# Manta-Network/Plonk-Prototype

Hardware: NVIDIA B200
Metric: PLONK prove time (BLS12-381 / KZG10, synthetic arithmetic circuit, 2^20 gates) (lower is better)
Workload: dtype u32 limbs (Fr 8x32, Fp 12x32)

## Files before the change

include/pb200.h:

```cpp
#ifndef PB200_H
#define PB200_H
#include <stddef.h>
#include <stdint.h>

#if defined(__GNUC__)
#define PB200_API __attribute__((visibility("default")))
#else
#define PB200_API
#endif

#ifdef __cplusplus
extern "C" {
#endif

typedef struct pb200_ctx pb200_ctx;
typedef struct pb200_srs pb200_srs;

enum {
    PB200_OK = 0,
    PB200_ERR_ARG = 1,
    PB200_ERR_CUDA = 2,
    PB200_ERR_NO_DEVICE = 3
};

PB200_API int pb200_init(pb200_ctx **out, int device_id);
PB200_API void pb200_destroy(pb200_ctx *ctx);
PB200_API const char *pb200_last_error(const pb200_ctx *ctx);
PB200_API void *pb200_stream(pb200_ctx *ctx);
PB200_API int pb200_sync(pb200_ctx *ctx);

PB200_API int pb200_malloc(pb200_ctx *ctx, void **dev_ptr, size_t bytes);
PB200_API int pb200_free(pb200_ctx *ctx, void *dev_ptr);
PB200_API int pb200_h2d(pb200_ctx *ctx, void *dev_dst, const void *host_src, size_t bytes);
PB200_API int pb200_d2h(pb200_ctx *ctx, void *host_dst, const void *dev_src, size_t bytes);

PB200_API int pb200_domain_log_size(size_t num_coeffs, uint32_t *log_n);
PB200_API int pb200_ntt(pb200_ctx *ctx, uint64_t *data_host, uint32_t log_n, int inverse, int coset);
PB200_API int pb200_ntt_dev(pb200_ctx *ctx, uint64_t *data_dev, uint32_t log_n, int inverse, int coset);

PB200_API int pb200_ntt_batch_dev(pb200_ctx *ctx, uint64_t *data_dev, uint32_t log_n, uint32_t batch, int inverse, int coset);
PB200_API int pb200_ntt_columns_dev(pb200_ctx *ctx, uint64_t *data_dev, uint32_t log_n, uint32_t log_n1, uint32_t log_cols,
                                    uint32_t col_offset, int inverse);
PB200_API int pb200_ntt_columns_scatter_dev(pb200_ctx *ctx, uint64_t *data_dev, uint32_t log_n, uint32_t log_n1, uint32_t log_cols,
                                            uint32_t col_offset, uint32_t world, void *const *peer_row_bufs);
PB200_API int pb200_ipc_export(pb200_ctx *ctx, void *dev_ptr, unsigned char handle_out[64]);
PB200_API int pb200_ipc_open(pb200_ctx *ctx, const unsigned char handle[64], void **dev_ptr_out);
PB200_API int pb200_ipc_close(pb200_ctx *ctx, void *dev_ptr);
PB200_API int pb200_block_transpose_dev(pb200_ctx *ctx, uint64_t *dst_dev, const uint64_t *src_dev, uint32_t blocks,
                                        uint32_t rows, uint32_t cols);

PB200_API int pb200_srs_upload(pb200_ctx *ctx, const uint64_t *xy_mont_host, size_t n_points, pb200_srs **out);
PB200_API int pb200_srs_wrap_dev(pb200_ctx *ctx, const uint64_t *xy_mont_dev, size_t n_points, pb200_srs **out);
PB200_API int pb200_srs_precompute(pb200_ctx *ctx, pb200_srs *srs);
PB200_API void pb200_srs_free(pb200_ctx *ctx, pb200_srs *srs);
PB200_API size_t pb200_srs_len(const pb200_srs *srs);
PB200_API int pb200_msm_g1(pb200_ctx *ctx, const pb200_srs *srs, size_t offset, const uint64_t *scalars_mont_host, size_t n,
                 uint64_t out_xyz_mont[18]);
PB200_API int pb200_msm_g1_dev(pb200_ctx *ctx, const pb200_srs *srs, size_t offset, const uint64_t *scalars_mont_dev, size_t n,
                     uint64_t out_xyz_mont[18]);
PB200_API int pb200_msm_g1_batch_dev(pb200_ctx *ctx, const pb200_srs *srs, size_t offset, const uint64_t *scalars_mont_dev, size_t n,
                                     uint32_t batch, size_t scalar_stride, uint64_t *out_xyz_mont);
PB200_API int pb200_pippenger_g1(pb200_ctx *ctx, const uint64_t *points_xyz_mont_host, const uint64_t *scalars_mont_host, size_t n,
                                 uint64_t out_xyz_mont[18]);
PB200_API int pb200_g1_sum(pb200_ctx *ctx, const uint64_t *points_xyz_mont_host, size_t count, uint64_t out_xyz_mont[18]);
PB200_API uint32_t pb200_msm_window_bits(size_t n);

PB200_API int pb200_srs_generate(pb200_ctx *ctx, const uint64_t tau_mont[4], size_t n_points, pb200_srs **out);
PB200_API int pb200_srs_generate_range(pb200_ctx *ctx, const uint64_t tau_mont[4], size_t first, size_t n_points, pb200_srs **out);
PB200_API const uint64_t *pb200_srs_dev_ptr(const pb200_srs *srs);
enum {
    PB200_G1_OK = 0,
    PB200_G1_BAD_FLAGS = 1,
    PB200_G1_X_RANGE = 2,
    PB200_G1_NOT_ON_CURVE = 3,
    PB200_G1_NOT_IN_SUBGROUP = 4,
    PB200_G1_IDENTITY = 5
};
PB200_API int pb200_srs_from_compressed(pb200_ctx *ctx, const uint8_t *bytes_host, size_t n_points, uint8_t *status_host,
                                        pb200_srs **out);
PB200_API int pb200_srs_to_compressed(pb200_ctx *ctx, const pb200_srs *srs, size_t offset, size_t n, uint8_t *bytes_host);
PB200_API int pb200_kzg_witness_dev(pb200_ctx *ctx, const uint64_t *poly_dev, size_t n, const uint64_t z_mont[4],
                                    uint64_t *quotient_dev, uint64_t eval_mont_out[4]);
PB200_API int pb200_fr_horner_step_dev(pb200_ctx *ctx, uint64_t *acc_dev, size_t n_acc, const uint64_t *poly_dev, size_t n_poly,
                                       const uint64_t c_mont[4]);

typedef struct pb200_prover_key pb200_prover_key;
// ... 69 lines not shown
```

plonk-prototype_b200/_native.py:

```python
import ctypes
import os

import numpy as np

_HERE = os.path.dirname(os.path.abspath(__file__))
LIB_PATH = os.path.join(_HERE, "libpb200.so")
_lib = None

EXPORTS = [
    "pb200_init", "pb200_destroy", "pb200_last_error", "pb200_stream", "pb200_sync",
    "pb200_malloc", "pb200_free", "pb200_h2d", "pb200_d2h",
    "pb200_domain_log_size", "pb200_ntt", "pb200_ntt_dev", "pb200_ntt_batch_dev", "pb200_ntt_columns_dev", "pb200_ntt_columns_scatter_dev",
    "pb200_ipc_export", "pb200_ipc_open", "pb200_ipc_close", "pb200_block_transpose_dev",
    "pb200_srs_upload", "pb200_srs_wrap_dev", "pb200_srs_precompute", "pb200_srs_free", "pb200_srs_len",
    "pb200_msm_g1", "pb200_msm_g1_dev", "pb200_msm_g1_batch_dev", "pb200_pippenger_g1", "pb200_g1_sum", "pb200_msm_window_bits",
    "pb200_srs_generate", "pb200_srs_generate_range", "pb200_srs_dev_ptr", "pb200_kzg_witness_dev", "pb200_fr_horner_step_dev",
    "pb200_srs_from_compressed", "pb200_srs_to_compressed",
    "pb200_preprocess", "pb200_preprocess_sharded", "pb200_prover_key_free", "pb200_prover_key_size", "pb200_prover_key_bytes", "pb200_prove", "pb200_prove_dev",
    "pb200_transcript_selftest", "pb200_synthetic_circuit", "pb200_verify", "pb200_verify_batch", "pb200_opening_key_from_tau",
    "pb200_pairing_selftest",
    "pb200_synthetic_bases_dev", "pb200_profile_enable", "pb200_profile_ms", "pb200_profile_reset", "pb200_profile_sum_ms",
    "pb200_launch_count",
    "pb200_imad_peak",
    "pb200_comm_unique_id", "pb200_comm_init", "pb200_comm_destroy", "pb200_comm_info", "pb200_allgather_dev", "pb200_alltoall_dev",
    "pb200_msm_g1_sharded_dev", "pb200_ntt_sharded_dev", "pb200_preprocess_comm",
]


class Pb200Error(RuntimeError):
    pass


G1_OK, G1_BAD_FLAGS, G1_X_RANGE, G1_NOT_ON_CURVE, G1_NOT_IN_SUBGROUP, G1_IDENTITY = range(6)


ALLGATHER_FN = ctypes.CFUNCTYPE(ctypes.c_int, ctypes.c_void_p, ctypes.c_void_p, ctypes.c_void_p, ctypes.c_size_t)
DEV_COLLECTIVE_FN = ctypes.CFUNCTYPE(ctypes.c_int, ctypes.c_void_p, ctypes.c_void_p, ctypes.c_void_p, ctypes.c_size_t)


class Shard(ctypes.Structure):
    _fields_ = [("rank", ctypes.c_uint32), ("world", ctypes.c_uint32), ("allgather", ALLGATHER_FN), ("user", ctypes.c_void_p),
                ("alltoall_dev", DEV_COLLECTIVE_FN), ("allgather_dev", DEV_COLLECTIVE_FN), ("flags", ctypes.c_uint32)]


class Circuit(ctypes.Structure):
    _fields_ = [("n_gates", ctypes.c_size_t), ("n_vars", ctypes.c_size_t), ("selectors", ctypes.c_void_p * 11),
                ("wires", ctypes.c_void_p * 4)]
# ... 3 lines not shown
    global _lib
    if _lib is None:
        if not os.path.exists(LIB_PATH):
            raise Pb200Error("libpb200.so is not built (run `python -c 'import __graft_entry__ as g; g.build()'`); "
                             "there is no CPU fallback")
        L = ctypes.CDLL(LIB_PATH)
        vp, u64p = ctypes.c_void_p, ctypes.c_void_p
        L.pb200_init.argtypes = [ctypes.POINTER(vp), ctypes.c_int]
        L.pb200_destroy.argtypes = [vp]
        L.pb200_destroy.restype = None
        L.pb200_last_error.argtypes = [vp]
        L.pb200_last_error.restype = ctypes.c_char_p
        L.pb200_stream.argtypes = [vp]
        L.pb200_stream.restype = vp
        L.pb200_sync.argtypes = [vp]
        L.pb200_malloc.argtypes = [vp, ctypes.POINTER(vp), ctypes.c_size_t]
        L.pb200_free.argtypes = [vp, vp]
        L.pb200_h2d.argtypes = [vp, vp, vp, ctypes.c_size_t]
        L.pb200_d2h.argtypes = [vp, vp, vp, ctypes.c_size_t]
        L.pb200_domain_log_size.argtypes = [ctypes.c_size_t, ctypes.POINTER(ctypes.c_uint32)]
        L.pb200_ntt.argtypes = [vp, u64p, ctypes.c_uint32, ctypes.c_int, ctypes.c_int]
        L.pb200_ntt_dev.argtypes = [vp, u64p, ctypes.c_uint32, ctypes.c_int, ctypes.c_int]
        L.pb200_ntt_batch_dev.argtypes = [vp, u64p, ctypes.c_uint32, ctypes.c_uint32, ctypes.c_int, ctypes.c_int]
        L.pb200_ntt_columns_dev.argtypes = [vp, u64p, ctypes.c_uint32, ctypes.c_uint32, ctypes.c_uint32, ctypes.c_uint32, ctypes.c_int]
        L.pb200_ntt_columns_scatter_dev.argtypes = [vp, u64p, ctypes.c_uint32, ctypes.c_uint32, ctypes.c_uint32, ctypes.c_uint32,
                                                    ctypes.c_uint32, ctypes.POINTER(vp)]
        L.pb200_ipc_export.argtypes = [vp, vp, ctypes.c_char_p]
        L.pb200_ipc_open.argtypes = [vp, ctypes.c_char_p, ctypes.POINTER(vp)]
        L.pb200_ipc_close.argtypes = [vp, vp]
        L.pb200_block_transpose_dev.argtypes = [vp, u64p, u64p, ctypes.c_uint32, ctypes.c_uint32, ctypes.c_uint32]
        L.pb200_srs_upload.argtypes = [vp, u64p, ctypes.c_size_t, ctypes.POINTER(vp)]
        L.pb200_srs_wrap_dev.argtypes = [vp, u64p, ctypes.c_size_t, ctypes.POINTER(vp)]
        L.pb200_srs_precompute.argtypes = [vp, vp]
        L.pb200_srs_free.argtypes = [vp, vp]
        L.pb200_srs_free.restype = None
        L.pb200_srs_len.argtypes = [vp]
        L.pb200_srs_len.restype = ctypes.c_size_t
        L.pb200_msm_g1.argtypes = [vp, vp, ctypes.c_size_t, u64p, ctypes.c_size_t, u64p]
        L.pb200_msm_g1_dev.argtypes = [vp, vp, ctypes.c_size_t, u64p, ctypes.c_size_t, u64p]
        L.pb200_msm_g1_batch_dev.argtypes = [vp, vp, ctypes.c_size_t, u64p, ctypes.c_size_t, ctypes.c_uint32, ctypes.c_size_t, u64p]
        L.pb200_g1_sum.argtypes = [vp, u64p, ctypes.c_size_t, u64p]
        L.pb200_pippenger_g1.argtypes = [vp, u64p, u64p, ctypes.c_size_t, u64p]
        L.pb200_msm_window_bits.argtypes = [ctypes.c_size_t]
        L.pb200_msm_window_bits.restype = ctypes.c_uint32
        L.pb200_srs_generate.argtypes = [vp, u64p, ctypes.c_size_t, ctypes.POINTER(vp)]
        L.pb200_srs_dev_ptr.argtypes = [vp]
        L.pb200_srs_dev_ptr.restype = vp
        L.pb200_kzg_witness_dev.argtypes = [vp, u64p, ctypes.c_size_t, u64p, u64p, u64p]
        L.pb200_fr_horner_step_dev.argtypes = [vp, u64p, ctypes.c_size_t, u64p, ctypes.c_size_t, u64p]
        L.pb200_preprocess.argtypes = [vp, vp, ctypes.POINTER(Circuit), ctypes.c_char_p, ctypes.c_size_t, ctypes.POINTER(vp), vp]
        L.pb200_preprocess_sharded.argtypes = [vp, vp, ctypes.POINTER(Circuit), ctypes.c_char_p, ctypes.c_size_t, ctypes.POINTER(Shard),
                                               ctypes.POINTER(vp), vp]
        L.pb200_srs_generate_range.argtypes = [vp, u64p, ctypes.c_size_t, ctypes.c_size_t, ctypes.POINTER(vp)]
        L.pb200_srs_from_compressed.argtypes = [vp, vp, ctypes.c_size_t, vp, ctypes.POINTER(vp)]
        L.pb200_srs_to_compressed.argtypes = [vp, vp, ctypes.c_size_t, ctypes.c_size_t, vp]
        L.pb200_prover_key_free.argtypes = [vp, vp]
        L.pb200_prover_key_free.restype = None
        L.pb200_prover_key_size.argtypes = [vp]
        L.pb200_prover_key_size.restype = ctypes.c_size_t
        L.pb200_prover_key_bytes.argtypes = [vp]
        L.pb200_prover_key_bytes.restype = ctypes.c_size_t
        L.pb200_prove.argtypes = [vp, vp, vp, u64p, vp, u64p, ctypes.c_size_t, vp]
        L.pb200_prove_dev.argtypes = [vp, vp, vp, u64p, vp, u64p, ctypes.c_size_t, vp]
        L.pb200_transcript_selftest.argtypes = [ctypes.c_char_p, ctypes.c_char_p, ctypes.c_char_p, ctypes.c_size_t, ctypes.c_char_p,
                                                ctypes.c_char_p, ctypes.c_size_t]
        L.pb200_verify.argtypes = [vp, ctypes.c_size_t, ctypes.c_char_p, ctypes.c_size_t, vp, vp, u64p, ctypes.c_size_t, u64p,
# ... 143 lines not shown
        self._check(lib().pb200_ntt_columns_scatter_dev(self._h, ctypes.c_void_p(dev), log_n, log_n1, log_cols, col_offset,
                                                        len(peer_row_bufs), arr))

    def ipc_export(self, dev):
        buf = ctypes.create_string_buffer(64)
        self._check(lib().pb200_ipc_export(self._h, ctypes.c_void_p(dev), buf))
        return buf.raw

    def ipc_open(self, handle):
        p = ctypes.c_void_p()
        self._check(lib().pb200_ipc_open(self._h, handle, ctypes.byref(p)))
        return p.value

    def ipc_close(self, dev):
        self._check(lib().pb200_ipc_close(self._h, ctypes.c_void_p(dev)))

    def block_transpose_dev(self, dst, src, blocks, rows, cols):
        self._check(lib().pb200_block_transpose_dev(self._h, ctypes.c_void_p(dst), ctypes.c_void_p(src), blocks, rows, cols))

    def srs_upload(self, xy_host):
        assert xy_host.dtype == np.uint64 and xy_host.size % 12 == 0
        h = ctypes.c_void_p()
        self._check(lib().pb200_srs_upload(self._h, _ptr(xy_host), xy_host.size // 12, ctypes.byref(h)))
        return h

    def srs_wrap_dev(self, dev, n):
        h = ctypes.c_void_p()
        self._check(lib().pb200_srs_wrap_dev(self._h, ctypes.c_void_p(dev), n, ctypes.byref(h)))
        return h

    def srs_precompute(self, srs):
        self._check(lib().pb200_srs_precompute(self._h, srs))

    def srs_free(self, srs):
        lib().pb200_srs_free(self._h, srs)

    def msm(self, srs, scalars_host, offset=0):
        n = scalars_host.size // 4
        out = np.zeros(18, np.uint64)
        self._check(lib().pb200_msm_g1(self._h, srs, offset, _ptr(scalars_host), n, _ptr(out)))
        return out

    def msm_dev(self, srs, scalars_dev, n, offset=0):
        out = np.zeros(18, np.uint64)
        self._check(lib().pb200_msm_g1_dev(self._h, srs, offset, ctypes.c_void_p(scalars_dev), n, _ptr(out)))
        return out

    def msm_batch_dev(self, srs, scalars_dev, n, batch, stride, offset=0):
        out = np.zeros((batch, 18), np.uint64)
        self._check(lib().pb200_msm_g1_batch_dev(self._h, srs, offset, ctypes.c_void_p(scalars_dev), n, batch, stride, _ptr(out)))
        return out

    def pippenger(self, points_xyz_host, scalars_host):
        pts = np.ascontiguousarray(points_xyz_host, dtype=np.uint64).reshape(-1, 18)
        sc = np.ascontiguousarray(scalars_host, dtype=np.uint64).reshape(-1, 4)
        assert pts.shape[0] == sc.shape[0]
        out = np.zeros(18, np.uint64)
        self._check(lib().pb200_pippenger_g1(self._h, _ptr(pts) if pts.size else None, _ptr(sc) if sc.size else None, pts.shape[0], _ptr(out)))
        return out

    def g1_sum(self, points_xyz_host):
        pts = np.ascontiguousarray(points_xyz_host, dtype=np.uint64).reshape(-1, 18)
        out = np.zeros(18, np.uint64)
        self._check(lib().pb200_g1_sum(self._h, _ptr(pts), pts.shape[0], _ptr(out)))
        return out

# ... 220 lines not shown
```

plonk-prototype_b200/csrc/common.cuh:

```cuda
#pragma once
#include <cuda_runtime.h>
#include <stdint.h>
#include <stdio.h>

#include <map>
#include <string>
#include <vector>

#include "../../include/pb200.h"

struct NttPlan;
struct pb200_comm;

struct pb200_ctx {
    int device = 0;
    int sm_count = 0;
    cudaStream_t stream = nullptr;
    std::string err;
    uint64_t launches = 0;
    bool profile = false;
    std::map<std::string, float> prof_ms;
    std::map<std::string, float> prof_sum;
    std::map<std::string, uint32_t> prof_cnt;
    std::map<uint32_t, NttPlan *> ntt_plans;
// ... 62 lines not shown
    void collect() {
        if (a && b) {
            float ms = 0;
            if (cudaEventElapsedTime(&ms, a, b) == cudaSuccess) {
                ctx->prof_ms[name] = ms;
                ctx->prof_sum[name] += ms;
                ctx->prof_cnt[name]++;
            }
            cudaEventDestroy(a);
            cudaEventDestroy(b);
            a = b = nullptr;
        }
    }
    ~PbTimer() {
        if (a) cudaEventDestroy(a);
        if (b) cudaEventDestroy(b);
    }
};

int pb_ensure(pb200_ctx *ctx, void **buf, size_t *have, size_t need);
int comm_allgather_host(pb200_ctx *ctx, const void *send, void *recv, size_t bytes);
int comm_stream_barrier(pb200_ctx *ctx);
uint32_t *comm_partials_buffer(pb200_ctx *ctx);
int comm_sum_partials(pb200_ctx *ctx, uint32_t batch, uint64_t *out_xyz_host);
struct pb200_srs;
int msm_batch_to_dev(pb200_ctx *ctx, const pb200_srs *srs, size_t offset, const uint64_t *scalars_dev, size_t n, uint32_t batch,
                     size_t scalar_stride, uint32_t *result_dev, bool *handled);
int tail_g1_sum_batch(pb200_ctx *ctx, const uint32_t *pts, uint32_t count, uint32_t batch, uint32_t *results);
int kzg_witness_slice_phase1(pb200_ctx *ctx, const uint64_t *poly_slice_dev, uint32_t lo, uint32_t cnt, const uint64_t z_mont[4],
                             uint64_t *q_slice_dev, uint64_t *work_dev, uint64_t slice_total_out[4]);
int kzg_witness_slice_phase2(pb200_ctx *ctx, uint32_t lo, uint32_t cnt, uint64_t *q_slice_dev, uint64_t *work_dev,
                             const uint64_t later_slices_total[4]);
size_t kzg_witness_slice_work_scalars(uint32_t cnt);
```

plonk-prototype_b200/csrc/host_field.h:

```cpp
#pragma once
#include <stdint.h>
#include <string.h>

namespace hostf {

typedef unsigned __int128 u128;

template <int N>
struct Params;

template <>
struct Params<4> {
    static constexpr uint64_t MOD[4] = {0xffffffff00000001ull, 0x53bda402fffe5bfeull, 0x3339d80809a1d805ull, 0x73eda753299d7d48ull};
    static constexpr uint64_t INV = 0xfffffffeffffffffull;
    static constexpr uint64_t R2[4] = {0xc999e990f3f29c6dull, 0x2b6cedcb87925c23ull, 0x05d314967254398full, 0x0748d9d99f59ff11ull};
};
template <>
struct Params<6> {
    static constexpr uint64_t MOD[6] = {0xb9feffffffffaaabull, 0x1eabfffeb153ffffull, 0x6730d2a0f6b0f624ull,
                                        0x64774b84f38512bfull, 0x4b1ba7b6434bacd7ull, 0x1a0111ea397fe69aull};
    static constexpr uint64_t INV = 0x89f3fffcfffcfffdull;
    static constexpr uint64_t R2[6] = {0xf4df1f341c341746ull, 0x0a76e6a609d104f1ull, 0x8de5476c4c95b6d5ull,
                                       0x67eb88a9939d83c0ull, 0x9a793e85b519952dull, 0x11988fe592cae3aaull};
};
// ... 98 lines not shown
                t[j - 1] = (uint64_t)c;
                c >>= 64;
            }
            c += t[N];
            t[N - 1] = (uint64_t)c;
            t[N] = t[N + 1] + (uint64_t)(c >> 64);
        }
        El r;
        memcpy(r.l, t, sizeof(r.l));
        if (t[N] || geq_mod(r.l)) sub_mod(r.l);
        return r;
    }
    El sqr() const { return *this * *this; }
    El from_mont() const { return *this * raw_u64(1); }
    El pow(const uint64_t *e, int words) const {
        El r = one();
        for (int i = words * 64 - 1; i >= 0; i--) {
            r = r.sqr();
            if ((e[i >> 6] >> (i & 63)) & 1) r = r * *this;
        }
        return r;
    }
    El pow_u64(uint64_t e) const { return pow(&e, 1); }
    El inv() const {
        uint64_t e[N];
        for (int i = 0; i < N; i++) e[i] = P::MOD[i];
        e[0] -= 2;
        return pow(e, N);
    }
};
typedef El<4> HFr;
typedef El<6> HFp;

inline void fr_to_bytes(const HFr &a, uint8_t out[32]) {
    HFr c = a.from_mont();
    for (int i = 0; i < 4; i++)
        for (int k = 0; k < 8; k++) out[8 * i + k] = (uint8_t)(c.l[i] >> (8 * k));
}
inline HFr fr_from_bytes_wide(const uint8_t in[64]) {
    HFr lo, hi;
    for (int i = 0; i < 4; i++) {
        lo.l[i] = hi.l[i] = 0;
        for (int k = 7; k >= 0; k--) {
            lo.l[i] = (lo.l[i] << 8) | in[8 * i + k];
            hi.l[i] = (hi.l[i] << 8) | in[32 + 8 * i + k];
        }
    }
    const HFr r2 = HFr::r2(), r3 = r2 * r2;
    return lo * r2 + hi * r3;
}
inline void g1_projective_to_bytes(const uint64_t xyz[18], uint8_t out[48]) {
    HFp X = HFp::load(xyz), Y = HFp::load(xyz + 6), Z = HFp::load(xyz + 12);
    memset(out, 0, 48);
    if (Z.is_zero()) {
        out[0] = 0xc0;
        return;
    }
    HFp zi = Z.inv();
    HFp x = (X * zi).from_mont(), y = (Y * zi).from_mont();
    for (int i = 0; i < 6; i++)
        for (int k = 0; k < 8; k++) out[47 - (8 * i + k)] = (uint8_t)(x.l[i] >> (8 * k));
    uint64_t d[7];
    uint64_t c = 0;
    for (int i = 0; i < 6; i++) {
        d[i] = (y.l[i] << 1) | c;
        c = y.l[i] >> 63;
// ... 7 lines not shown
```

plonk-prototype_b200/csrc/plonk.cu:

```cuda
#include <algorithm>
#include <chrono>
#include <cstdlib>
#include <cstring>
#include <vector>

#include "common.cuh"
#include "fr_vec.cuh"
#include "host_field.h"
#include "merlin.h"
#include "widgets.h"

using hostf::HFr;

namespace {

constexpr int kSel = 11;
enum { Q_M, Q_L, Q_R, Q_O, Q_C, Q_4, Q_ARITH, Q_RANGE, Q_LOGIC, Q_FIXED, Q_VAR };
const char *const kSelLabel[kSel] = {"q_m", "q_l", "q_r", "q_o", "q_c", "q_4", "q_arith", "q_range", "q_logic",
                                     "q_fixed_group_add", "q_variable_group_add"};
const int kSeedOrder[kSel] = {Q_M, Q_L, Q_R, Q_O, Q_C, Q_4, Q_ARITH, Q_RANGE, Q_LOGIC, Q_VAR, Q_FIXED};

inline Fr to_dev(const HFr &h) {
    Fr r;
    memcpy(r.l, h.l, 32);
// ... 301 lines not shown
    if (first < len) {
        const uint32_t last = min(first + kEvalPerThread, len);
        acc = ld_fr(p + last - 1);
        for (uint32_t j = last - 1; j-- > first;) acc = acc * x + ld_fr(p + j);
        acc = acc * x.pow_u32(A.off[job] + first);
    }
    acc = block_sum(acc, sm);
    if (threadIdx.x == 0) st_fr(A.partial + (size_t)job * A.tiles + blockIdx.x, acc);
}
__global__ void __launch_bounds__(256) poly_eval_final_kernel(const Fr *partial, uint32_t tiles, Fr *out) {
    __shared__ uint4 smraw[512];
    Fr *sm = reinterpret_cast<Fr *>(smraw);
    const uint32_t job = blockIdx.x;
    Fr acc = Fr::zero();
    for (uint32_t t = threadIdx.x; t < tiles; t += 256) acc = acc + ld_fr(partial + (size_t)job * tiles + t);
    acc = block_sum(acc, sm);
    if (threadIdx.x == 0) st_fr(out + job, acc);
}

inline uint32_t cdiv(size_t a, uint32_t b) { return (uint32_t)((a + b - 1) / b); }

}

struct pb200_prover_key {
    uint32_t log_n = 0;
    size_t n = 0, n_gates = 0, n_vars = 0;
    bool q_nonzero[kSel] = {};
    void *slab = nullptr;
    size_t slab_bytes = 0;
    Fr *q_poly[kSel] = {}, *q_4n[kSel] = {};
    Fr *sig_evals = nullptr, *sig_poly = nullptr, *sig_4n = nullptr;
    Fr *roots = nullptr, *lin_4n = nullptr, *l1_4n = nullptr;
    uint32_t *wires = nullptr;
    Fr *values = nullptr, *w_evals = nullptr, *w_poly = nullptr, *z_poly = nullptr, *pi_poly = nullptr, *ev4 = nullptr, *t_poly = nullptr,
       *lin_poly = nullptr, *agg = nullptr, *wit = nullptr, *num = nullptr, *den = nullptr, *small = nullptr;
    uint32_t *pi_pos = nullptr;
    size_t pi_cap = 0;
    HFr vh_inv[4];
    HFr omega, omega4;
    uint8_t vk_bytes[15 * 48];
    merlin::Transcript *seeded = nullptr;
    pb200_shard shard = {0, 1, nullptr, nullptr, nullptr, nullptr, 0};
    size_t slice_lo = 0, slice_n = 0;
    void *peer_slab[8] = {};
    bool peers_open = false, peers_failed = false;
};

namespace {

struct Carver {
    char *base;
    size_t off = 0;
    explicit Carver(void *b) : base((char *)b) {}
    template <class T>
    T *take(size_t count) {
        T *p = base ? (T *)(base + off) : nullptr;
        off += (count * sizeof(T) + 255) & ~(size_t)255;
        return p;
    }
};
inline size_t scan_tiles(size_t n) { return (n + kTile - 1) / kTile; }
inline size_t eval_tiles(size_t n4) { return (n4 + kEvalTile - 1) / kEvalTile; }

void carve(pb200_prover_key *pk, void *base, size_t *total) {
    Carver c(base);
    const size_t n = pk->n, N4 = 4 * n;
// ... 97 lines not shown
    for (int k = 0; k < count; k++) {
        HFr acc = HFr::zero();
        for (uint32_t r = 0; r < world; r++) acc = acc + HFr::load(&all[((size_t)r * count + k) * 4]);
        out[k] = acc;
    }
    return 0;
}

struct RoundClock {
    pb200_ctx *ctx;
    std::chrono::steady_clock::time_point t0;
    explicit RoundClock(pb200_ctx *c) : ctx(c), t0(std::chrono::steady_clock::now()) {}
    void lap(const char *name) {
        if (!ctx->profile) return;
        cudaStreamSynchronize(ctx->stream);
        auto t1 = std::chrono::steady_clock::now();
        const float ms = std::chrono::duration<float, std::milli>(t1 - t0).count();
        ctx->prof_ms[name] = ms;
        ctx->prof_sum[name] += ms;
        ctx->prof_cnt[name]++;
        t0 = t1;
    }
};

}

extern "C" void pb200_prover_key_free(pb200_ctx *ctx, pb200_prover_key *pk) {
    if (!pk) return;
    if (ctx) cudaSetDevice(ctx->device);
    for (uint32_t h = 0; h < 8; h++)
        if (pk->peer_slab[h] && h != pk->shard.rank) cudaIpcCloseMemHandle(pk->peer_slab[h]);
    cudaFree(pk->slab);
    cudaFree(pk->pi_pos);
    delete pk->seeded;
    delete pk;
}
extern "C" size_t pb200_prover_key_size(const pb200_prover_key *pk) { return pk ? pk->n : 0; }
extern "C" size_t pb200_prover_key_bytes(const pb200_prover_key *pk) { return pk ? pk->slab_bytes : 0; }

extern "C" int pb200_preprocess(pb200_ctx *ctx, const pb200_srs *srs, const pb200_circuit *circuit, const uint8_t *transcript_label,
                                size_t label_len, pb200_prover_key **out, uint8_t vk_commitments[15 * 48]) {
    return pb200_preprocess_sharded(ctx, srs, circuit, transcript_label, label_len, nullptr, out, vk_commitments);
}
extern "C" int pb200_preprocess_sharded(pb200_ctx *ctx, const pb200_srs *srs, const pb200_circuit *circuit,
                                        const uint8_t *transcript_label, size_t label_len, const pb200_shard *shard,
                                        pb200_prover_key **out, uint8_t vk_commitments[15 * 48]) {
    if (!ctx) return PB200_ERR_ARG;
    const uint32_t world = shard ? shard->world : 1;
    PB_ARG(ctx, world >= 1 && (world & (world - 1)) == 0 && (world == 1 || (shard->allgather != nullptr && shard->rank < world)));
    PB_ARG(ctx, srs != nullptr && circuit != nullptr && out != nullptr && (transcript_label != nullptr || label_len == 0));
    PB_ARG(ctx, circuit->n_gates >= 1 && circuit->n_vars >= 1 && circuit->n_vars < ((size_t)1 << 32));
    for (int c = 0; c < 4; c++) PB_ARG(ctx, circuit->wires[c] != nullptr);
    uint32_t log_n = 0;
    PB_TRY(pb200_domain_log_size(circuit->n_gates, &log_n));
    PB_ARG(ctx, log_n <= 26);
    const size_t n = (size_t)1 << log_n, N4 = 4 * n, ng = circuit->n_gates;
    PB_ARG(ctx, world <= n && pb200_srs_len(srs) >= n / world);
    PB_CUDA(ctx, cudaSetDevice(ctx->device));

    pb200_prover_key *pk = new pb200_prover_key();
    if (world > 1) pk->shard = *shard;
    pk->slice_n = n / world;
    pk->slice_lo = (size_t)pk->shard.rank * pk->slice_n;
    pk->log_n = log_n;
    pk->n = n;
    pk->n_gates = ng;
    pk->n_vars = circuit->n_vars;
    auto fail = [&](int rc) {
        pb200_prover_key_free(ctx, pk);
        return rc;
    };
// ... 24 lines not shown
            }
        for (size_t v = 0; v < circuit->n_vars; v++)
            if (last[v] != none) map[(size_t)(last[v] >> log_n) * n + (last[v] & (n - 1))] = first[v];
    }
    carve(pk, nullptr, &pk->slab_bytes);
    cudaError_t e = cudaMalloc(&pk->slab, pk->slab_bytes);
    if (e != cudaSuccess) {
        pb_fail(ctx, PB200_ERR_CUDA, "prover key allocation", cudaGetErrorString(e), __FILE__, __LINE__);
        return fail(PB200_ERR_CUDA);
    }
    size_t dummy;
    carve(pk, pk->slab, &dummy);
    cudaStream_t st = ctx->stream;
#define PK_CUDA(call)                                                                                         \
    do {                                                                                                      \
        cudaError_t e__ = (call);                                                                             \
        if (e__ != cudaSuccess) {                                                                             \
            pb_fail(ctx, PB200_ERR_CUDA, #call, cudaGetErrorString(e__), __FILE__, __LINE__);                 \
            return fail(PB200_ERR_CUDA);                                                                      \
        }                                                                                                     \
    } while (0)
#define PK_TRY(expr)                    \
    do {                                \
        int rc__ = (expr);              \
        if (rc__) return fail(rc__);    \
    } while (0)
#define PK_LAUNCHED()                                                                                         \
    do {                                                                                                      \
        ctx->launches++;                                                                                      \
        PK_CUDA(cudaGetLastError());                                                                          \
    } while (0)

    {
        uint64_t root32[4] = {0xb9b58d8c5f0e466aull, 0x5b1b4c801819d7ecull, 0x0af53ae352a31e64ull, 0x5bf3adda19e9b27bull};
        HFr w = HFr::load(root32);
        HFr w4 = w;
        for (uint32_t k = 0; k < 32 - log_n; k++) w = w.sqr();
        for (uint32_t k = 0; k < 32 - (log_n + 2); k++) w4 = w4.sqr();
        pk->omega = w;
        pk->omega4 = w4;
        const HFr g = HFr::from_u64(7), gn = g.pow_u64(n), i4 = w4.pow_u64(n), one = HFr::one();
        HFr cur = gn;
        for (int k = 0; k < 4; k++) {
            pk->vh_inv[k] = (cur - one).inv();
            cur = cur * i4;
        }
    }
    KFactors ks;
    ks.k[0] = to_dev(HFr::one());
    ks.k[1] = to_dev(HFr::from_u64(7));
    ks.k[2] = to_dev(HFr::from_u64(13));
    ks.k[3] = to_dev(HFr::from_u64(17));

    for (int c = 0; c < 4; c++)
        PK_CUDA(cudaMemcpyAsync(pk->wires + (size_t)c * ng, circuit->wires[c], ng * 4, cudaMemcpyHostToDevice, st));
    uint32_t *map_dev = (uint32_t *)pk->t_poly;
    PK_CUDA(cudaMemcpyAsync(map_dev, map.data(), 4 * n * 4, cudaMemcpyHostToDevice, st));
    powers_kernel<<<cdiv(n, 256), 256, 0, st>>>(pk->roots, (uint32_t)n, to_dev(HFr::one()), to_dev(pk->omega));
    PK_LAUNCHED();
    powers_kernel<<<cdiv(N4, 256), 256, 0, st>>>(pk->lin_4n, (uint32_t)N4, to_dev(HFr::from_u64(7)), to_dev(pk->omega4));
    PK_LAUNCHED();
    sigma_evals_kernel<<<dim3(cdiv(n, 256), 4), 256, 0, st>>>(pk->sig_evals, map_dev, pk->roots, (uint32_t)n, log_n, ks);
    PK_LAUNCHED();
    PK_CUDA(cudaStreamSynchronize(st));

    uint8_t *vk = pk->vk_bytes;
    {
        int first = -1;
        uint32_t n_sel = 0;
        for (int s = 0; s < kSel; s++) {
            uint8_t *dst = vk + 48 * s;
            memset(dst, 0, 48);
            dst[0] = 0xc0;
            if (!pk->q_nonzero[s]) continue;
            if (first < 0) first = s;
            n_sel++;
            PK_CUDA(cudaMemsetAsync(pk->q_poly[s], 0, n * sizeof(Fr), st));
            PK_CUDA(cudaMemcpyAsync(pk->q_poly[s], circuit->selectors[s], ng * sizeof(Fr), cudaMemcpyHostToDevice, st));
        }
        if (n_sel) {
            uint8_t packed[kSel * 48];
            PK_TRY(pb200_ntt_batch_dev(ctx, (uint64_t *)pk->q_poly[first], log_n, n_sel, 1, 0));
            PK_TRY(commit_bytes_batch(ctx, srs, pk, pk->q_poly[first], n, n_sel, n, packed));
            PK_TRY(coset_extend(ctx, pk->q_4n[first], pk->q_poly[first], (uint32_t)n, log_n + 2, n_sel));
            for (int s = 0, k = 0; s < kSel; s++)
                if (pk->q_nonzero[s]) memcpy(vk + 48 * s, packed + 48 * k++, 48);
        }
    }
    PK_CUDA(cudaMemcpyAsync(pk->sig_poly, pk->sig_evals, 4 * n * sizeof(Fr), cudaMemcpyDeviceToDevice, st));
    PK_TRY(pb200_ntt_batch_dev(ctx, (uint64_t *)pk->sig_poly, log_n, 4, 1, 0));
    PK_TRY(commit_bytes_batch(ctx, srs, pk, pk->sig_poly, n, 4, n, vk + 48 * kSel));
    PK_TRY(coset_extend(ctx, pk->sig_4n, pk->sig_poly, (uint32_t)n, log_n + 2, 4));
    fill_kernel<<<cdiv(n, 256), 256, 0, st>>>(pk->lin_poly, (uint32_t)n, to_dev(HFr::from_u64(n).inv()));
    PK_LAUNCHED();
    PK_TRY(coset_extend(ctx, pk->l1_4n, pk->lin_poly, (uint32_t)n, log_n + 2, 1));
    PK_CUDA(cudaStreamSynchronize(st));

    pk->seeded = new merlin::Transcript(transcript_label, label_len);
    for (int k = 0; k < kSel; k++) pk->seeded->append_commitment(kSelLabel[kSeedOrder[k]], vk + 48 * kSeedOrder[k]);
    const char *const sig_label[4] = {"left_sigma", "right_sigma", "out_sigma", "fourth_sigma"};
    for (int c = 0; c < 4; c++) pk->seeded->append_commitment(sig_label[c], vk + 48 * (kSel + c));
    pk->seeded->circuit_domain_sep(n);
    if (vk_commitments) memcpy(vk_commitments, vk, sizeof(pk->vk_bytes));
    *out = pk;
    return 0;
#undef PK_CUDA
#undef PK_TRY
#undef PK_LAUNCHED
}

static int prove_impl(pb200_ctx *ctx, const pb200_srs *srs, pb200_prover_key *pk, const uint64_t *values_mont, bool values_on_device,
                      const uint32_t *pi_gate, const uint64_t *pi_mont, size_t n_pi, uint8_t proof_out[1040]);
extern "C" int pb200_prove(pb200_ctx *ctx, const pb200_srs *srs, pb200_prover_key *pk, const uint64_t *values_mont,
                           const uint32_t *pi_gate, const uint64_t *pi_mont, size_t n_pi, uint8_t proof_out[1040]) {
    return prove_impl(ctx, srs, pk, values_mont, false, pi_gate, pi_mont, n_pi, proof_out);
}
extern "C" int pb200_prove_dev(pb200_ctx *ctx, const pb200_srs *srs, pb200_prover_key *pk, const uint64_t *values_mont_dev,
                               const uint32_t *pi_gate, const uint64_t *pi_mont, size_t n_pi, uint8_t proof_out[1040]) {
    return prove_impl(ctx, srs, pk, values_mont_dev, true, pi_gate, pi_mont, n_pi, proof_out);
}
static int prove_impl(pb200_ctx *ctx, const pb200_srs *srs, pb200_prover_key *pk, const uint64_t *values_mont, bool values_on_device,
                      const uint32_t *pi_gate, const uint64_t *pi_mont, size_t n_pi, uint8_t proof_out[1040]) {
    if (!ctx) return PB200_ERR_ARG;
    PB_ARG(ctx, srs != nullptr && pk != nullptr && values_mont != nullptr && proof_out != nullptr);
    PB_ARG(ctx, n_pi == 0 || (pi_gate != nullptr && pi_mont != nullptr));
    PB_ARG(ctx, pb200_srs_len(srs) >= pk->slice_n);
    for (size_t j = 0; j < n_pi; j++) PB_ARG(ctx, pi_gate[j] < pk->n);
    if (n_pi > 1) {
        std::vector<uint32_t> sorted(pi_gate, pi_gate + n_pi);
        std::sort(sorted.begin(), sorted.end());
        PB_ARG(ctx, std::adjacent_find(sorted.begin(), sorted.end()) == sorted.end());
    }
    PB_CUDA(ctx, cudaSetDevice(ctx->device));
    cudaStream_t st = ctx->stream;
    const size_t n = pk->n, N4 = 4 * n;
    const uint32_t n32 = (uint32_t)n, log_n = pk->log_n;
    RoundClock clk(ctx);
    merlin::Transcript tr = *pk->seeded;
    uint8_t *P = proof_out;
    KFactors ks;
    ks.k[0] = to_dev(HFr::one());
    ks.k[1] = to_dev(HFr::from_u64(7));
    ks.k[2] = to_dev(HFr::from_u64(13));
    ks.k[3] = to_dev(HFr::from_u64(17));
    Fr *scal = pk->small;
    Fr *tilesA = pk->small + 64, *tilesB = tilesA + scan_tiles(n), *partial = tilesB + scan_tiles(n);

    const Fr *values_dev = (const Fr *)values_mont;
    if (!values_on_device) {
        PB_CUDA(ctx, cudaMemcpyAsync(pk->values, values_mont, pk->n_vars * sizeof(Fr), cudaMemcpyHostToDevice, st));
        values_dev = pk->values;
    }
    gather_wires_kernel<<<dim3(cdiv(n, 256), 4), 256, 0, st>>>(pk->w_evals, pk->wires, values_dev, (uint32_t)pk->n_gates, n32);
    PB_LAUNCHED(ctx);
    PB_CUDA(ctx, cudaMemcpyAsync(pk->w_poly, pk->w_evals, 4 * n * sizeof(Fr), cudaMemcpyDeviceToDevice, st));
    PB_TRY(pb200_ntt_batch_dev(ctx, (uint64_t *)pk->w_poly, log_n, 4, 1, 0));
    const char *const w_label[4] = {"w_l", "w_r", "w_o", "w_4"};
    PB_TRY(commit_bytes_batch(ctx, srs, pk, pk->w_poly, n, 4, n, P));
    for (int c = 0; c < 4; c++) tr.append_commitment(w_label[c], P + 48 * c);
    clk.lap("prove.round1");

    const HFr beta = tr.challenge_scalar("beta");
    tr.append_scalar("beta", beta);
    const HFr gamma = tr.challenge_scalar("gamma");
    perm_numden_kernel<<<cdiv(n, 256), 256, 0, st>>>(pk->w_evals, pk->sig_evals, pk->roots, n32, to_dev(beta), to_dev(gamma), ks, pk->num,
                                                    pk->den);
    PB_LAUNCHED(ctx);
    PB_TRY(launch_scan(ctx, pk, pk->num, n32, false, tilesA, scal + 0));
    PB_TRY(launch_scan(ctx, pk, pk->den, n32, true, tilesB, scal + 1));
    fr_inv_kernel<<<1, 1, 0, st>>>(scal + 1, scal + 2);
    PB_LAUNCHED(ctx);
    perm_finish_kernel<<<cdiv(n, 256), 256, 0, st>>>(pk->num, pk->den, scal + 2, n32, pk->z_poly);
    PB_LAUNCHED(ctx);
    PB_TRY(pb200_ntt_dev(ctx, (uint64_t *)pk->z_poly, log_n, 1, 0));
    PB_TRY(commit_bytes(ctx, srs, pk, pk->z_poly, n, P + 48 * 4));
    tr.append_commitment("z", P + 48 * 4);
    clk.lap("prove.round2");

    const HFr alpha = tr.challenge_scalar("alpha");
    const HFr range_sep = tr.challenge_scalar("range separation challenge");
    const HFr logic_sep = tr.challenge_scalar("logic separation challenge");
    const HFr fixed_sep = tr.challenge_scalar("fixed base separation challenge");
    const HFr var_sep = tr.challenge_scalar("variable base separation challenge");
    const HFr edwards_d = (HFr::from_u64(10240) * HFr::from_u64(10241).inv()).neg();
    PB_CUDA(ctx, cudaMemsetAsync(pk->pi_poly, 0, n * sizeof(Fr), st));
    if (n_pi) {
        if (pk->pi_cap < n_pi) {
            cudaFree(pk->pi_pos);
            pk->pi_pos = nullptr;
            pk->pi_cap = 0;
            PB_CUDA(ctx, cudaMalloc((void **)&pk->pi_pos, n_pi * (4 + sizeof(Fr)) + 32));
// ... 430 lines not shown
```

Before: 79.97.

## Commit wire polynomials from evaluations using a precomputed Lagrange-basis SRS

Adds a Lagrange-basis commitment key, built at preprocess time by running an inverse FFT over the G1 SRS points on the GPU and then normalising them to affine. When that key exists, the round-1 wire commitments take their MSM over the wire evaluations directly instead of over the interpolated coefficients. The inverse NTT into w_poly still runs because later rounds need it, so the saving comes only from the MSM input path and any change in scalar distribution. In exchange preprocessing gets slower and uses more memory, since the key has its own precompute tables.

```diff
diff --git a/include/pb200.h b/include/pb200.h
--- a/include/pb200.h
+++ b/include/pb200.h
@@ -52,6 +52,7 @@
 PB200_API int pb200_srs_upload(pb200_ctx *ctx, const uint64_t *xy_mont_host, size_t n_points, pb200_srs **out);
 PB200_API int pb200_srs_wrap_dev(pb200_ctx *ctx, const uint64_t *xy_mont_dev, size_t n_points, pb200_srs **out);
 PB200_API int pb200_srs_precompute(pb200_ctx *ctx, pb200_srs *srs);
+PB200_API int pb200_srs_lagrange(pb200_ctx *ctx, const pb200_srs *srs, uint32_t log_n, pb200_srs **out);
 PB200_API void pb200_srs_free(pb200_ctx *ctx, pb200_srs *srs);
 PB200_API size_t pb200_srs_len(const pb200_srs *srs);
 PB200_API int pb200_msm_g1(pb200_ctx *ctx, const pb200_srs *srs, size_t offset, const uint64_t *scalars_mont_host, size_t n,
diff --git a/plonk-prototype_b200/_native.py b/plonk-prototype_b200/_native.py
--- a/plonk-prototype_b200/_native.py
+++ b/plonk-prototype_b200/_native.py
@@ -12,7 +12,7 @@
     "pb200_malloc", "pb200_free", "pb200_h2d", "pb200_d2h",
     "pb200_domain_log_size", "pb200_ntt", "pb200_ntt_dev", "pb200_ntt_batch_dev", "pb200_ntt_columns_dev", "pb200_ntt_columns_scatter_dev",
     "pb200_ipc_export", "pb200_ipc_open", "pb200_ipc_close", "pb200_block_transpose_dev",
-    "pb200_srs_upload", "pb200_srs_wrap_dev", "pb200_srs_precompute", "pb200_srs_free", "pb200_srs_len",
+    "pb200_srs_upload", "pb200_srs_wrap_dev", "pb200_srs_precompute", "pb200_srs_lagrange", "pb200_srs_free", "pb200_srs_len",
     "pb200_msm_g1", "pb200_msm_g1_dev", "pb200_msm_g1_batch_dev", "pb200_pippenger_g1", "pb200_g1_sum", "pb200_msm_window_bits",
     "pb200_srs_generate", "pb200_srs_generate_range", "pb200_srs_dev_ptr", "pb200_kzg_witness_dev", "pb200_fr_horner_step_dev",
     "pb200_srs_from_compressed", "pb200_srs_to_compressed",
@@ -82,6 +82,7 @@
         L.pb200_srs_upload.argtypes = [vp, u64p, ctypes.c_size_t, ctypes.POINTER(vp)]
         L.pb200_srs_wrap_dev.argtypes = [vp, u64p, ctypes.c_size_t, ctypes.POINTER(vp)]
         L.pb200_srs_precompute.argtypes = [vp, vp]
+        L.pb200_srs_lagrange.argtypes = [vp, vp, ctypes.c_uint32, ctypes.POINTER(vp)]
         L.pb200_srs_free.argtypes = [vp, vp]
         L.pb200_srs_free.restype = None
         L.pb200_srs_len.argtypes = [vp]
@@ -291,6 +292,11 @@
     def srs_precompute(self, srs):
         self._check(lib().pb200_srs_precompute(self._h, srs))
 
+    def srs_lagrange(self, srs, log_n):
+        h = ctypes.c_void_p()
+        self._check(lib().pb200_srs_lagrange(self._h, srs, log_n, ctypes.byref(h)))
+        return h
+
     def srs_free(self, srs):
         lib().pb200_srs_free(self._h, srs)
 
diff --git a/plonk-prototype_b200/csrc/common.cuh b/plonk-prototype_b200/csrc/common.cuh
--- a/plonk-prototype_b200/csrc/common.cuh
+++ b/plonk-prototype_b200/csrc/common.cuh
@@ -118,3 +118,4 @@
 int kzg_witness_slice_phase2(pb200_ctx *ctx, uint32_t lo, uint32_t cnt, uint64_t *q_slice_dev, uint64_t *work_dev,
                              const uint64_t later_slices_total[4]);
 size_t kzg_witness_slice_work_scalars(uint32_t cnt);
+int lagrange_srs_build(pb200_ctx *ctx, const pb200_srs *srs, uint32_t log_n, pb200_srs **out, bool *degenerate);
diff --git a/plonk-prototype_b200/csrc/host_field.h b/plonk-prototype_b200/csrc/host_field.h
--- a/plonk-prototype_b200/csrc/host_field.h
+++ b/plonk-prototype_b200/csrc/host_field.h
@@ -154,6 +154,12 @@
 typedef El<4> HFr;
 typedef El<6> HFp;
 
+inline HFr domain_root(uint32_t log_n) {
+    const uint64_t root32[4] = {0xb9b58d8c5f0e466aull, 0x5b1b4c801819d7ecull, 0x0af53ae352a31e64ull, 0x5bf3adda19e9b27bull};
+    HFr w = HFr::load(root32);
+    for (uint32_t k = log_n; k < 32; k++) w = w.sqr();
+    return w;
+}
 inline void fr_to_bytes(const HFr &a, uint8_t out[32]) {
     HFr c = a.from_mont();
     for (int i = 0; i < 4; i++)
diff --git a/plonk-prototype_b200/csrc/lagrange.cu b/plonk-prototype_b200/csrc/lagrange.cu
--- /dev/null
+++ b/plonk-prototype_b200/csrc/lagrange.cu
@@ -0,0 +1,85 @@
+#define PB_FIELD_NOINLINE_MUL 1
+#include "common.cuh"
+#include "host_field.h"
+#include "lagrange.cuh"
+
+namespace {
+
+__global__ void __launch_bounds__(128) lagrange_load_kernel(const G1Affine *__restrict__ bases, uint32_t log_n, G1Xyzz *a) {
+    const uint32_t i = blockIdx.x * blockDim.x + threadIdx.x;
+    if (i < (1u << log_n)) lagrange::load_point(bases, i, log_n, a);
+}
+__global__ void __launch_bounds__(128) lagrange_stage_kernel(G1Xyzz *a, uint32_t n, uint32_t half, Fr w) {
+    const uint32_t k = blockIdx.x * blockDim.x + threadIdx.x;
+    if (k < n / 2) lagrange::butterfly(a, half, k, w);
+}
+__global__ void __launch_bounds__(128) lagrange_normalize_kernel(G1Xyzz *a, uint32_t n, Fr n_inv, G1Affine *out, uint32_t *degenerate) {
+    const uint32_t i0 = (blockIdx.x * blockDim.x + threadIdx.x) * lagrange::kNormPer;
+    if (i0 < n) lagrange::normalize(a, i0, min(lagrange::kNormPer, n - i0), n_inv, out, degenerate);
+}
+
+inline Fr to_dev(const hostf::HFr &h) {
+    Fr r;
+    memcpy(r.l, h.l, 32);
+    return r;
+}
+
+}
+
+int lagrange_srs_build(pb200_ctx *ctx, const pb200_srs *srs, uint32_t log_n, pb200_srs **out, bool *degenerate) {
+    *out = nullptr;
+    *degenerate = false;
+    PB_ARG(ctx, srs != nullptr && srs->dev != nullptr && log_n <= 26 && ((size_t)1 << log_n) <= srs->n);
+    PB_CUDA(ctx, cudaSetDevice(ctx->device));
+    const uint32_t n = 1u << log_n;
+    cudaStream_t st = ctx->stream;
+    void *work = nullptr, *pts = nullptr;
+    PB_CUDA(ctx, cudaMalloc(&work, (size_t)n * sizeof(G1Xyzz) + 256));
+    cudaError_t e = cudaMalloc(&pts, (size_t)n * sizeof(G1Affine));
+    G1Xyzz *a = (G1Xyzz *)work;
+    uint32_t *flag = (uint32_t *)((char *)work + (size_t)n * sizeof(G1Xyzz));
+    uint32_t flag_host = 0;
+    if (e == cudaSuccess) e = cudaMemsetAsync(flag, 0, 4, st);
+    if (e == cudaSuccess) {
+        lagrange_load_kernel<<<(n + 127) / 128, 128, 0, st>>>((const G1Affine *)srs->dev, log_n, a);
+        ctx->launches++;
+        e = cudaGetLastError();
+    }
+    const hostf::HFr w_inv = hostf::domain_root(log_n).inv();
+    for (uint32_t half = 1; half < n && e == cudaSuccess; half <<= 1) {
+        lagrange_stage_kernel<<<(n / 2 + 127) / 128, 128, 0, st>>>(a, n, half, to_dev(w_inv.pow_u64(n / (2 * half))));
+        ctx->launches++;
+        e = cudaGetLastError();
+    }
+    if (e == cudaSuccess) {
+        const uint32_t threads = (n + lagrange::kNormPer - 1) / lagrange::kNormPer;
+        lagrange_normalize_kernel<<<(threads + 127) / 128, 128, 0, st>>>(a, n, to_dev(hostf::HFr::from_u64(n).inv()), (G1Affine *)pts, flag);
+        ctx->launches++;
+        e = cudaGetLastError();
+    }
+    if (e == cudaSuccess) e = cudaMemcpyAsync(&flag_host, flag, 4, cudaMemcpyDeviceToHost, st);
+    if (e == cudaSuccess) e = cudaStreamSynchronize(st);
+    cudaFree(work);
+    if (e != cudaSuccess || flag_host) {
+        cudaFree(pts);
+        if (e != cudaSuccess) return pb_fail(ctx, PB200_ERR_CUDA, "lagrange commit key", cudaGetErrorString(e), __FILE__, __LINE__);
+        *degenerate = true;
+        return 0;
+    }
+    pb200_srs *s = new pb200_srs();
+    s->dev = (const uint64_t *)pts;
+    s->n = n;
+    s->owned = true;
+    *out = s;
+    return 0;
+}
+
+extern "C" int pb200_srs_lagrange(pb200_ctx *ctx, const pb200_srs *srs, uint32_t log_n, pb200_srs **out) {
+    if (!ctx) return PB200_ERR_ARG;
+    PB_ARG(ctx, out != nullptr);
+    bool degenerate = false;
+    PB_TRY(lagrange_srs_build(ctx, srs, log_n, out, &degenerate));
+    if (degenerate) return pb_fail(ctx, PB200_ERR_ARG, "lagrange commit key", "a Lagrange point is the identity: the key is not powers of tau",
+                                   __FILE__, __LINE__);
+    return 0;
+}
diff --git a/plonk-prototype_b200/csrc/lagrange.cuh b/plonk-prototype_b200/csrc/lagrange.cuh
--- /dev/null
+++ b/plonk-prototype_b200/csrc/lagrange.cuh
@@ -0,0 +1,68 @@
+#pragma once
+#include "g1.cuh"
+
+namespace lagrange {
+
+constexpr uint32_t kNormPer = 8;
+
+PB_HD uint32_t bitrev(uint32_t i, uint32_t bits) {
+    uint32_t r = 0;
+    for (uint32_t b = 0; b < bits; b++) r |= ((i >> b) & 1u) << (bits - 1 - b);
+    return r;
+}
+PB_HD G1Xyzz g1_neg(const G1Xyzz &p) {
+    G1Xyzz r = p;
+    r.y = p.y.neg();
+    return r;
+}
+PB_HD G1Xyzz g1_mul_fr(const G1Xyzz &p, const Fr &k_mont) {
+    const Fr k = k_mont.from_mont();
+    int top = 255;
+    while (top >= 0 && !((k.l[top >> 5] >> (top & 31)) & 1)) top--;
+    if (top < 0) return G1Xyzz::identity();
+    G1Xyzz acc = p;
+    for (int i = top - 1; i >= 0; i--) {
+        acc = g1_dbl(acc);
+        if ((k.l[i >> 5] >> (i & 31)) & 1) acc = g1_add(acc, p);
+    }
+    return acc;
+}
+
+PB_HD void load_point(const G1Affine *bases, uint32_t i, uint32_t log_n, G1Xyzz *a) {
+    a[bitrev(i, log_n)] = G1Xyzz::from_affine(bases[i]);
+}
+PB_HD void butterfly(G1Xyzz *a, uint32_t half, uint32_t k, const Fr &w) {
+    const uint32_t j = k & (half - 1), i0 = ((k - j) << 1) + j, i1 = i0 + half;
+    const G1Xyzz u = a[i0];
+    G1Xyzz t = a[i1];
+    if (j) t = g1_mul_fr(t, w.pow_u32(j));
+    a[i0] = g1_add(u, t);
+    a[i1] = g1_add(u, g1_neg(t));
+}
+PB_HD void normalize(G1Xyzz *a, uint32_t i0, uint32_t cnt, const Fr &n_inv, G1Affine *out, uint32_t *degenerate) {
+    Fp prefix[kNormPer];
+    Fp run = Fp::one();
+    for (uint32_t k = 0; k < cnt; k++) {
+        const G1Xyzz p = g1_mul_fr(a[i0 + k], n_inv);
+        a[i0 + k] = p;
+        prefix[k] = run;
+        if (!p.is_identity()) run = run * (p.zz * p.zzz);
+    }
+    Fp inv = run.inv();
+    for (int k = (int)cnt - 1; k >= 0; k--) {
+        const G1Xyzz p = a[i0 + k];
+        G1Affine r;
+        if (p.is_identity()) {
+            r.x = r.y = Fp::zero();
+            *degenerate = 1;
+        } else {
+            const Fp zi = inv * prefix[k];
+            inv = inv * (p.zz * p.zzz);
+            r.x = p.x * (zi * p.zzz);
+            r.y = p.y * (zi * p.zz);
+        }
+        out[i0 + k] = r;
+    }
+}
+
+}
diff --git a/plonk-prototype_b200/csrc/plonk.cu b/plonk-prototype_b200/csrc/plonk.cu
--- a/plonk-prototype_b200/csrc/plonk.cu
+++ b/plonk-prototype_b200/csrc/plonk.cu
@@ -357,6 +357,8 @@
     Fr *sig_evals = nullptr, *sig_poly = nullptr, *sig_4n = nullptr;
     Fr *roots = nullptr, *lin_4n = nullptr, *l1_4n = nullptr;
     uint32_t *wires = nullptr;
+    pb200_srs *lagrange = nullptr;
+    size_t lagrange_bytes = 0;
     Fr *values = nullptr, *w_evals = nullptr, *w_poly = nullptr, *z_poly = nullptr, *pi_poly = nullptr, *ev4 = nullptr, *t_poly = nullptr,
        *lin_poly = nullptr, *agg = nullptr, *wit = nullptr, *num = nullptr, *den = nullptr, *small = nullptr;
     uint32_t *pi_pos = nullptr;
@@ -520,11 +522,12 @@
         if (pk->peer_slab[h] && h != pk->shard.rank) cudaIpcCloseMemHandle(pk->peer_slab[h]);
     cudaFree(pk->slab);
     cudaFree(pk->pi_pos);
+    pb200_srs_free(ctx, pk->lagrange);
     delete pk->seeded;
     delete pk;
 }
 extern "C" size_t pb200_prover_key_size(const pb200_prover_key *pk) { return pk ? pk->n : 0; }
-extern "C" size_t pb200_prover_key_bytes(const pb200_prover_key *pk) { return pk ? pk->slab_bytes : 0; }
+extern "C" size_t pb200_prover_key_bytes(const pb200_prover_key *pk) { return pk ? pk->slab_bytes + pk->lagrange_bytes : 0; }
 
 extern "C" int pb200_preprocess(pb200_ctx *ctx, const pb200_srs *srs, const pb200_circuit *circuit, const uint8_t *transcript_label,
                                 size_t label_len, pb200_prover_key **out, uint8_t vk_commitments[15 * 48]) {
@@ -615,12 +618,8 @@
     } while (0)
 
     {
-        uint64_t root32[4] = {0xb9b58d8c5f0e466aull, 0x5b1b4c801819d7ecull, 0x0af53ae352a31e64ull, 0x5bf3adda19e9b27bull};
-        HFr w = HFr::load(root32);
-        HFr w4 = w;
-        for (uint32_t k = 0; k < 32 - log_n; k++) w = w.sqr();
-        for (uint32_t k = 0; k < 32 - (log_n + 2); k++) w4 = w4.sqr();
-        pk->omega = w;
+        const HFr w4 = hostf::domain_root(log_n + 2);
+        pk->omega = hostf::domain_root(log_n);
         pk->omega4 = w4;
         const HFr g = HFr::from_u64(7), gn = g.pow_u64(n), i4 = w4.pow_u64(n), one = HFr::one();
         HFr cur = gn;
@@ -678,6 +677,16 @@
     PK_LAUNCHED();
     PK_TRY(coset_extend(ctx, pk->l1_4n, pk->lin_poly, (uint32_t)n, log_n + 2, 1));
     PK_CUDA(cudaStreamSynchronize(st));
+
+    const char *lag_env = getenv("PB200_LAGRANGE_COMMIT");
+    if (world == 1 && log_n <= 22 && srs->pre != nullptr && !(lag_env && strcmp(lag_env, "0") == 0)) {
+        bool degenerate = false;
+        PK_TRY(lagrange_srs_build(ctx, srs, log_n, &pk->lagrange, &degenerate));
+        if (pk->lagrange) {
+            PK_TRY(pb200_srs_precompute(ctx, pk->lagrange));
+            pk->lagrange_bytes = n * 96 * (1 + pk->lagrange->W_pre);
+        }
+    }
 
     pk->seeded = new merlin::Transcript(transcript_label, label_len);
     for (int k = 0; k < kSel; k++) pk->seeded->append_commitment(kSelLabel[kSeedOrder[k]], vk + 48 * kSeedOrder[k]);
@@ -739,7 +748,8 @@
     PB_CUDA(ctx, cudaMemcpyAsync(pk->w_poly, pk->w_evals, 4 * n * sizeof(Fr), cudaMemcpyDeviceToDevice, st));
     PB_TRY(pb200_ntt_batch_dev(ctx, (uint64_t *)pk->w_poly, log_n, 4, 1, 0));
     const char *const w_label[4] = {"w_l", "w_r", "w_o", "w_4"};
-    PB_TRY(commit_bytes_batch(ctx, srs, pk, pk->w_poly, n, 4, n, P));
+    if (pk->lagrange) PB_TRY(commit_bytes_batch(ctx, pk->lagrange, pk, pk->w_evals, n, 4, n, P));
+    else PB_TRY(commit_bytes_batch(ctx, srs, pk, pk->w_poly, n, 4, n, P));
     for (int c = 0; c < 4; c++) tr.append_commitment(w_label[c], P + 48 * c);
     clk.lap("prove.round1");
 
```

Result: faster. 74.85, median of 6 (-6.4%).
